# UmbertoDellaMonica/fp-mash

Measured on AMD Instinct MI355X. Metric: bases/s sketched + Mpairs/s dist, k=21 s=1000, 1/2/4/8 MI355X; %HBM roofline, higher is better.
Workload: dtype u64; 1 GPU; n_seqs_per_gpu=10000, seq_len=2000, k=21, s=1000, pairs_per_gpu=100000000, listed_pairs_per_gpu=1000006, full=False

## Files before the change

### fp-mash_amd/csrc/sketch.hip

```cpp
#include "fpm_device.hpp"
#include "fpm_kernels.hpp"
#include "screen_table.hpp"

namespace fpm {

constexpr int kBlock = 256;
constexpr int kSkWpe = 7;
constexpr int kSkWpeThr = 8;
constexpr int kWaves = kBlock / 64;

#ifdef FPM_SKETCH_PHASES
__device__ uint64_t *g_phase;
#define FPM_PHASE_DECL uint64_t ph_[8] = {0, 0, 0, 0, 0, 0, 0, 0}
#define FPM_PHASE(i) do { if (threadIdx.x == 0) ph_[i] = __builtin_amdgcn_s_memtime(); } while (0)
#define FPM_PHASE_FLUSH do { if (threadIdx.x == 0) for (int q_ = 0; q_ < 8; q_++) g_phase[blockIdx.x * 8 + q_] = ph_[q_]; } while (0)
#else
#define FPM_PHASE_DECL do {} while (0)
#define FPM_PHASE(i) do {} while (0)
#define FPM_PHASE_FLUSH do {} while (0)
#endif

__device__ __forceinline__ uint32_t block_exscan(uint32_t v, uint32_t *tmp, uint32_t *total)
{
    const int lane = threadIdx.x & 63, wave = threadIdx.x >> 6;
// ... 9 lines not shown
        uint32_t acc = 0;
        for (int w = 0; w < kWaves; w++) { uint32_t t = tmp[w]; tmp[w] = acc; acc += t; }
        tmp[kWaves] = acc;
    }
    __syncthreads();
    uint32_t ex = tmp[wave] + x - v;
    *total = tmp[kWaves];
    __syncthreads();
    return ex;
}

__device__ __forceinline__ uint32_t lane_prefix(uint64_t m)
{
    return __builtin_amdgcn_mbcnt_hi((uint32_t)(m >> 32), __builtin_amdgcn_mbcnt_lo((uint32_t)m, 0u));
}

template <int P>
__device__ __forceinline__ void write_distinct(const uint64_t *keys, uint32_t nv, uint64_t *row,
                                               uint32_t s, uint32_t *wcnt, uint32_t *total, int tid)
{
    constexpr int E = P / kBlock;
    constexpr int NW = E * kWaves;
    constexpr int PL = (NW + 63) / 64;
    const int lane = tid & 63, wave = tid >> 6;
#pragma unroll
    for (int e = 0; e < E; e++) {
        const uint32_t i = (uint32_t)(e * kBlock + tid);
        const bool f = i < nv && (i == 0 || keys[i] != keys[i - 1]);
        const uint64_t m = __ballot(f);
        if (lane == 0) wcnt[e * kWaves + wave] = (uint32_t)__popcll(m);
    }
    __syncthreads();
    if (tid < 64) {
        uint32_t v[PL], sum = 0;
#pragma unroll
        for (int q = 0; q < PL; q++) {
            const int i = tid * PL + q;
            v[q] = i < NW ? wcnt[i] : 0u;
            sum += v[q];
        }
        uint32_t x = sum;
#pragma unroll
        for (int d = 1; d < 64; d <<= 1) {
            const uint32_t y = __shfl_up(x, d, 64);
            if (lane >= d) x += y;
        }
        uint32_t ex = x - sum;
#pragma unroll
        for (int q = 0; q < PL; q++) {
            const int i = tid * PL + q;
            if (i < NW) wcnt[i] = ex;
            ex += v[q];
        }
        if (tid == 63) wcnt[NW] = x;
    }
    __syncthreads();
    *total = wcnt[NW];
#pragma unroll
    for (int e = 0; e < E; e++) {
        const uint32_t i = (uint32_t)(e * kBlock + tid);
        const uint64_t key = i < nv ? keys[i] : 0ULL;
        const bool f = i < nv && (i == 0 || key != keys[i - 1]);
        const uint64_t m = __ballot(f);
        const uint32_t rank = wcnt[e * kWaves + wave] + lane_prefix(m);
        if (f && rank < s) row[rank] = key;
    }
}

template <int P>
__device__ void bitonic_sort(uint64_t *keys)
{
    const int tid = threadIdx.x;
    for (int ks = 2; ks <= P; ks <<= 1) {
        for (int j = ks >> 1; j > 0; j >>= 1) {
            for (int t = tid; t < P / 2; t += kBlock) {
                int i = ((t & ~(j - 1)) << 1) | (t & (j - 1));
                int l = i + j;
                bool up = (i & ks) == 0;
                uint64_t a = keys[i], b = keys[l];
                if ((a > b) == up) { keys[i] = b; keys[l] = a; }
            }
            __syncthreads();
        }
    }
}

__device__ __forceinline__ uint32_t upper4(uint32_t x)
{
    const uint32_t hi = x & 0x80808080u, lo = x & 0x7f7f7f7fu;
    const uint32_t ge = (lo + 0x1f1f1f1fu) & ~hi;
    const uint32_t le = ~(lo + 0x05050505u) & ~hi;
    const uint32_t m = (ge & le & 0x80808080u) >> 2;
    return x - m;
}

__device__ __forceinline__ uint32_t compl4(uint32_t x)
{
    const uint32_t b1 = (x >> 1) & 0x01010101u;
    return x ^ (b1 * 0x04u + (b1 ^ 0x01010101u) * 0x15u);
}

template <int P>
struct TileImg {
    static constexpr int E = P / kBlock;
    static constexpr int kRcPad = ((E + 15) / 16) * 16;
    static constexpr int kFBytes = ((P + 31 + 15 + 96 + 31) / 32) * 32;
    static constexpr int kRBytes = ((kRcPad + P + 31 + 15 + 96 + 15) / 16) * 16;
    static constexpr int kMaskWords = kFBytes / 32 + 2;
    static constexpr int kBytes = kFBytes + kRBytes + 4 * kMaskWords + 512;
};

template <int P>
__device__ __forceinline__ void tile_stage(const uint8_t *__restrict__ seq, const TileDesc &td,
                                           const SketchKParams &p, uint32_t *img, int tid)
{
    using I = TileImg<P>;
    uint32_t *const fwd_img = img;
    uint32_t *const rc_img = fwd_img + I::kFBytes / 4;
    uint32_t *const badmask = rc_img + I::kRBytes / 4;
    const uint8_t *const alpha = reinterpret_cast<const uint8_t *>(badmask + I::kMaskWords);
    const uint8_t *const compl_tab = alpha + 256;
    const uint32_t n = td.n_bytes;
    const uint32_t a0 = (uint32_t)(td.byte_off & 15);
    const uint8_t *g0 = seq + (td.byte_off - a0);
    const uint32_t nimg = a0 + n;
    const uint32_t rc0 = I::kRcPad + ((16u - (nimg & 15u)) & 15u);
    constexpr int kChunks = I::kFBytes / 16;
    for (int ch = tid; ch < kChunks; ch += kBlock) {
        const uint32_t y0 = (uint32_t)ch * 16;
        uint4 v = make_uint4(0, 0, 0, 0);
        if (y0 < nimg) v = *reinterpret_cast<const uint4 *>(g0 + y0);
        uint32_t w[4] = {v.x, v.y, v.z, v.w};
        uint32_t bad = 0;
#pragma unroll
        for (int q = 0; q < 4; q++) {
            if (!p.preserve_case) w[q] = upper4(w[q]);
#pragma unroll
            for (int b = 0; b < 4; b++) {
                const uint32_t y = y0 + 4 * q + b;
                const bool ok = y >= a0 && y < nimg && alpha[(w[q] >> (8 * b)) & 0xffu];
                bad |= (ok ? 0u : 1u) << (4 * q + b);
            }
        }
        *reinterpret_cast<uint4 *>(&fwd_img[y0 / 4]) = make_uint4(w[0], w[1], w[2], w[3]);
        if (p.canonical && y0 < nimg) {
            const uint32_t zc = rc0 + nimg - 16 - y0;
            uint32_t c[4];
            if (p.compl_acgt) {
#pragma unroll
                for (int q = 0; q < 4; q++) c[q] = compl4(w[q]);
            } else {
#pragma unroll
                for (int q = 0; q < 4; q++) {
                    uint32_t x = 0;
#pragma unroll
                    for (int b = 0; b < 4; b++)
                        x |= (uint32_t)compl_tab[(w[q] >> (8 * b)) & 0xffu] << (8 * b);
                    c[q] = x;
                }
            }
            *reinterpret_cast<uint4 *>(&rc_img[zc / 4]) =
                make_uint4(__builtin_bswap32(c[3]), __builtin_bswap32(c[2]),
                           __builtin_bswap32(c[1]), __builtin_bswap32(c[0]));
        }
        const uint32_t hi = __shfl_down(bad, 1, 64);
        if ((ch & 1) == 0) badmask[ch / 2] = bad | (hi << 16);
    }
    if (tid < 2) badmask[I::kMaskWords - 2 + tid] = 0xffffffffu;
}

template <int P, int K, typename Sink>
__device__ __forceinline__ uint32_t tile_hash(const TileDesc &td, const SketchKParams &p,
                                              const uint32_t *img, int tid, Sink &&sink)
{
    using I = TileImg<P>;
    constexpr int E = I::E;
    const uint32_t *const fwd_img = img;
    const uint32_t *const rc_img = fwd_img + I::kFBytes / 4;
    const uint32_t *const badmask = rc_img + I::kRBytes / 4;
    const uint32_t n = td.n_bytes;
    const uint32_t k = K ? (uint32_t)K : p.k;
    const uint32_t a0 = (uint32_t)(td.byte_off & 15);
    const uint32_t nimg = a0 + n;
    const uint32_t rc0 = I::kRcPad + ((16u - (nimg & 15u)) & 15u);
    const uint32_t nk = n >= k ? n - k + 1 : 0;
    const int nw = (k + 3) >> 2;
    const uint32_t tail_mask = (k & 3) ? ((1u << (8 * (k & 3))) - 1u) : 0xffffffffu;
    const uint32_t kmask = (k == 32) ? 0xffffffffu : ((1u << k) - 1u);
    constexpr int KW = K ? (K + 3) / 4 : 8;
    constexpr int W = (E + 3) / 4 + KW + 1;
    uint32_t vbits = 0;
    uint32_t seed;
    asm volatile("s_mov_b32 %0, %1" : "=s"(seed) : "s"(p.seed));
    const uint32_t i0 = (uint32_t)tid * E;
    if (i0 < nk) {
        const uint32_t yb = a0 + i0;
        uint32_t okbits = 0;
        {
            const uint32_t wq = yb >> 5, sh = yb & 31;
            uint64_t bits = ((uint64_t)badmask[wq] | ((uint64_t)badmask[wq + 1] << 32)) >> sh;
            if (sh) bits |= (uint64_t)badmask[wq + 2] << (64 - sh);
#pragma unroll
            for (int e = 0; e < E; e++) {
                const bool ok = i0 + e < nk && (((uint32_t)(bits >> e) & kmask) == 0);
                okbits |= (ok ? 1u : 0u) << e;
            }
        }
        if (okbits) {
            uint32_t S[W];
            {
                const uint32_t q0 = yb >> 2, sh0 = yb & 3;
                uint32_t D[W + 1];
#pragma unroll
                for (int m = 0; m <= W; m++) D[m] = fwd_img[q0 + m];
#pragma unroll
                for (int m = 0; m < W; m++) S[m] = __builtin_amdgcn_alignbyte(D[m + 1], D[m], sh0);
            }
            uint32_t SR[W];
            if (p.canonical) {
                const uint32_t zb = rc0 + n - i0 - k - (E - 1);
                const uint32_t qr = zb >> 2, shr = zb & 3;
                uint32_t D[W + 1];
#pragma unroll
                for (int m = 0; m <= W; m++) D[m] = rc_img[qr + m];
#pragma unroll
                for (int m = 0; m < W; m++) SR[m] = __builtin_amdgcn_alignbyte(D[m + 1], D[m], shr);
            }
#pragma unroll
            for (int e = 0; e < E; e++) {
                if (!(okbits >> e & 1)) continue;
                uint32_t d[8];
#pragma unroll
                for (int m = 0; m < 8; m++)
                    d[m] = (m < nw) ? __builtin_amdgcn_alignbyte(S[(e >> 2) + m + 1], S[(e >> 2) + m],
                                                                 e & 3)
                                    : 0u;
                d[nw - 1] &= tail_mask;
                if (p.canonical) {
                    const int f = E - 1 - e;
                    uint32_t r[8];
#pragma unroll
                    for (int m = 0; m < 8; m++)
                        r[m] = (m < nw) ? __builtin_amdgcn_alignbyte(SR[(f >> 2) + m + 1],
                                                                     SR[(f >> 2) + m], f & 3)
                                        : 0u;
                    r[nw - 1] &= tail_mask;
                    constexpr int NQ = K ? ((K + 3) / 4 + 1) / 2 : 4;
                    bool gt = false, eq = true;
#pragma unroll
                    for (int q = 0; q < NQ; q++) {
                        const uint64_t fq = ((uint64_t)__builtin_bswap32(d[2 * q]) << 32) |
                                            __builtin_bswap32(d[2 * q + 1]);
                        const uint64_t rq = ((uint64_t)__builtin_bswap32(r[2 * q]) << 32) |
                                            __builtin_bswap32(r[2 * q + 1]);
                        gt = gt || (eq && fq > rq);
                        eq = eq && fq == rq;
                    }
                    const int cmp = gt ? 1 : 0;
                    if (cmp > 0) {
#pragma unroll
                        for (int m = 0; m < 8; m++) d[m] = r[m];
                    }
                }
                uint64_t wd[4];
#pragma unroll
                for (int j = 0; j < 4; j++) wd[j] = (uint64_t)d[2 * j] | ((uint64_t)d[2 * j + 1] << 32);
                const uint64_t h = murmur_h1_le32(wd, (int)k, seed);
                sink(e, p.use64 ? h : (h & 0xffffffffULL));
            }
            vbits = okbits;
        }
    }
    return vbits;
}

constexpr int kSurv = 2;
constexpr int kSurvShared = 512;
static_assert(kBlock * kSurv + kSurvShared == (int)kThrTileKeys, "sketch_plan.cpp sizes thr4 by it");
template <int P, int K, bool THR>
__device__ __forceinline__ void sketch_tile(
    const uint8_t *__restrict__ seq, const TileDesc td, SketchKParams p,
    const uint64_t *__restrict__ thr, uint64_t *__restrict__ out, uint32_t *__restrict__ out_count,
    TileDesc *__restrict__ redo, uint32_t *__restrict__ redo_n)
{
    using I = TileImg<P>;
    constexpr int E = I::E;
    constexpr int PS = THR ? kBlock * kSurv + kSurvShared : P;
    constexpr int ES = PS / kBlock;
    constexpr int KW = THR ? (PS > (I::kBytes + 7) / 8 ? PS : (I::kBytes + 7) / 8) : P;
    __shared__ __attribute__((aligned(16))) uint64_t keys[KW];
    static_assert(I::kBytes <= 8 * KW, "staging fits in keys");
    constexpr int kBins = P >= 4096 ? P / 4 : P / 2;
    static_assert(!THR || kBins <= 2 * (kBlock * kSurv + kSurvShared), "bins fit the slots");
    __shared__ uint64_t surv[THR ? kBlock * kSurv + kSurvShared : 1];
    __shared__ uint32_t s_over, s_shared;
    uint32_t *const img = reinterpret_cast<uint32_t *>(keys);
    uint8_t *const alpha = reinterpret_cast<uint8_t *>(img + (I::kFBytes + I::kRBytes) / 4 +
                                                       I::kMaskWords);
    uint8_t *const compl_tab = alpha + 256;
    __shared__ uint32_t scan_tmp[kWaves + 1];
    __shared__ uint32_t wcnt[ES * kWaves + 1];
    __shared__ uint32_t bins_own[THR ? 1 : kBins];
    uint32_t *const bins = THR ? reinterpret_cast<uint32_t *>(surv) : bins_own;
    __shared__ uint32_t big_bucket, s_cut;

    FPM_PHASE_DECL;
    FPM_PHASE(0);
    const int tid = threadIdx.x;

    alpha[tid] = p.alphabet[tid];
    compl_tab[tid] = p.complement[tid];
    if (THR && tid == 0) { s_over = 0; s_shared = 0; }
    __syncthreads();

    tile_stage<P>(seq, td, p, img, tid);
    __syncthreads();
    FPM_PHASE(1);

    uint64_t kr[ES];
    uint32_t vbits;
    uint64_t hmax = p.use64 ? ~0ULL : 0xffffffffULL;
    if constexpr (THR) {
        hmax = min(hmax, thr[td.thr_slot - 1]);
        uint32_t ns = 0;
        tile_hash<P, K>(td, p, img, tid, [&](int, uint64_t h) {
            if (h <= hmax) {
                if (ns < (uint32_t)kSurv) {
                    surv[tid * kSurv + ns] = h;
                    ns++;
                } else {
                    const uint32_t j = atomicAdd(&s_shared, 1u);
                    if (j < (uint32_t)kSurvShared) surv[kBlock * kSurv + j] = h;
                    else s_over = 1;
                }
            }
        });
        uint32_t total;
        uint32_t at = block_exscan(ns, scan_tmp, &total);
        if (s_over) {
            if (tid == 0) redo[atomicAdd(redo_n, 1u)] = td;
            return;
        }
        for (uint32_t i = 0; i < ns; i++) keys[at + i] = surv[tid * kSurv + i];
        const uint32_t nsh = s_shared;
        for (uint32_t i = tid; i < nsh; i += kBlock) keys[total + i] = surv[kBlock * kSurv + i];
        total += nsh;
        __syncthreads();
        if (total <= 64) {
            if (tid < 64) {
                const uint64_t v = tid < total ? keys[tid] : 0;
                const uint32_t vlo = (uint32_t)v, vhi = (uint32_t)(v >> 32);
                bool first = tid < total;
#pragma unroll 1
                for (uint32_t j = 0; j < total; j++) {
                    const uint64_t y = ((uint64_t)(uint32_t)__builtin_amdgcn_readlane((int)vhi, (int)j) << 32) |
                                       (uint32_t)__builtin_amdgcn_readlane((int)vlo, (int)j);
                    first = first && !(j < tid && y == v);
                }
                const uint64_t fm = __builtin_amdgcn_ballot_w64(first);
                uint32_t rank = 0;
#pragma unroll 1
                for (uint32_t j = 0; j < total; j++) {
                    const uint64_t y = ((uint64_t)(uint32_t)__builtin_amdgcn_readlane((int)vhi, (int)j) << 32) |
                                       (uint32_t)__builtin_amdgcn_readlane((int)vlo, (int)j);
                    rank += ((fm >> j) & 1) && y < v ? 1u : 0u;
                }
                if (first && rank < p.s) out[(uint64_t)td.out_row * p.s + rank] = v;
                if (tid == 0) {
                    const uint32_t nd = (uint32_t)__popcll(fm);
                    out_count[td.out_row] = nd < p.s ? nd : p.s;
                }
            }
            return;
        }
        vbits = 0;
#pragma unroll
        for (int e = 0; e < ES; e++) {
            const uint32_t j = (uint32_t)tid + (uint32_t)e * kBlock;
            kr[e] = ~0ULL;
            if (j < total) { kr[e] = keys[j]; vbits |= 1u << e; }
        }
        __syncthreads();
    } else {
#pragma unroll
    for (int e = 0; e < E; e++) kr[e] = ~0ULL;
    vbits = tile_hash<P, K>(td, p, img, tid, [&](int e, uint64_t h) { kr[e] = h; });

    FPM_PHASE(2);
    if (td.thr_slot) {
        hmax = min(hmax, thr[td.thr_slot - 1]);
#pragma unroll
        for (int e = 0; e < E; e++)
            if (kr[e] > hmax) vbits &= ~(1u << e);
        if (E > 1) {
            uint32_t total;
            uint32_t at = block_exscan((uint32_t)__popc(vbits), scan_tmp, &total);
            if (total <= (uint32_t)(kBlock * (E / 2))) {
#pragma unroll
                for (int e = 0; e < E; e++)
                    if (vbits >> e & 1) keys[at++] = kr[e];
                __syncthreads();
                vbits = 0;
#pragma unroll
                for (int e = 0; e < E; e++) {
                    const uint32_t j = (uint32_t)tid + (uint32_t)e * kBlock;
                    if (j < total) { kr[e] = keys[j]; vbits |= 1u << e; }
                }
                __syncthreads();
            }
        }
    }
    }

    constexpr int NB = P >= 4096 ? P / 4 : P / 2;
    constexpr int LB = __builtin_ctz(NB);
    constexpr uint32_t kMaxBucket = 32;
    const uint32_t hbits = hmax ? 64 - __clzll(hmax) : 1;
    const uint32_t bshift = hbits > (uint32_t)LB ? hbits - LB : 0;
    for (int b = tid; b < NB; b += kBlock) bins[b] = 0;
    if (tid == 0) { big_bucket = 0; s_cut = NB; }
    __syncthreads();
#pragma unroll
    for (int e = 0; e < ES; e++)
        if (vbits >> e & 1) atomicAdd(&bins[(uint32_t)(kr[e] >> bshift)], 1u);
    __syncthreads();
    FPM_PHASE(3);
    constexpr int per = NB >= kBlock ? NB / kBlock : 1;
    uint32_t run = 0, bmax = 0;
#pragma unroll
    for (int u = 0; u < per; u++) {
        const int b = tid * per + u;
        const uint32_t c = b < NB ? bins[b] : 0u;
        run += c;
        bmax = max(bmax, c);
    }
    uint32_t nvalid;
    uint32_t acc = block_exscan(run, scan_tmp, &nvalid);
#pragma unroll
    for (int u = 0; u < per; u++) {
        const int b = tid * per + u;
        if (b < NB) {
            const uint32_t c = bins[b];
            bins[b] = acc;
            if (acc < p.s && acc + c >= p.s) s_cut = (uint32_t)b + 1;
            acc += c;
        }
    }
    if (bmax > kMaxBucket) big_bucket = 1;
    __syncthreads();
    const uint32_t cut = big_bucket ? (uint32_t)NB : s_cut;
    const uint32_t nkept = cut < (uint32_t)NB ? bins[cut] : nvalid;
    FPM_PHASE(4);
    uint32_t lo_b = 0, hi_b = cut, nv = nkept;
    for (int pass = 0; pass < 2; pass++) {
        uint32_t bsh = bshift;
        asm volatile("" : "+v"(bsh));
        uint32_t act = 0;
#pragma unroll
        for (int e = 0; e < ES; e++) {
            const uint32_t bk = (uint32_t)(kr[e] >> bsh);
            act |= ((vbits >> e & 1) && bk >= lo_b && bk < hi_b) ? (1u << e) : 0u;
        }
        uint32_t slot[ES];
#pragma unroll
        for (int e = 0; e < ES; e++)
            if (act >> e & 1) {
                slot[e] = atomicAdd(&bins[(uint32_t)(kr[e] >> bsh)], 1u);
                keys[slot[e]] = kr[e];
            }
        __syncthreads();
        FPM_PHASE(5);
        if (!big_bucket) {
#pragma unroll
            for (int e = 0; e < ES; e++)
                if (act >> e & 1) {
                    const uint32_t b = (uint32_t)(kr[e] >> bsh);
                    const uint32_t s0 = b ? bins[b - 1] : 0u, s1 = bins[b];
                    const uint32_t mb = s1 - s0;
                    uint32_t r = 0;
#pragma unroll
                    for (uint32_t u = 0; u < 8; u++) {
                        const uint32_t t = s0 + u;
                        const uint64_t y = keys[t < (uint32_t)PS ? t : (uint32_t)PS - 1];
                        r += (u < mb) & ((y < kr[e]) | ((y == kr[e]) & (t < slot[e])));
                    }
                    for (uint32_t t = s0 + 8; t < s1; t++) {
                        const uint64_t y = keys[t];
                        r += (y < kr[e]) | ((y == kr[e]) & (t < slot[e]));
                    }
                    slot[e] = s0 + r;
                }
            __syncthreads();
#pragma unroll
            for (int e = 0; e < ES; e++)
                if (act >> e & 1) keys[slot[e]] = kr[e];
            __syncthreads();
        } else {
            for (int i = tid; i < PS; i += kBlock)
                if ((uint32_t)i >= nvalid) keys[i] = ~0ULL;
            __syncthreads();
            bitonic_sort<PS>(keys);
        }
        FPM_PHASE(6);

        uint32_t total;
        write_distinct<PS>(keys, nv, out + (uint64_t)td.out_row * p.s, p.s, wcnt, &total, tid);
        if (total >= p.s || hi_b >= (uint32_t)NB) {
            if (tid == 0) out_count[td.out_row] = total < p.s ? total : p.s;
            break;
        }
        lo_b = hi_b;
        hi_b = NB;
        nv = nvalid;
    }
    FPM_PHASE(7);
    FPM_PHASE_FLUSH;
}

template <int P, int K, bool THR = false>
__global__ __launch_bounds__(kBlock) __attribute__((amdgpu_waves_per_eu(THR ? (K ? kSkWpeThr : 6) : P <= 2048 ? kSkWpe : P == 4096 ? 4 : 1))) void sketch_tiles_kernel(
    const uint8_t *__restrict__ seq, const TileDesc *__restrict__ tiles, SketchKParams p,
    const uint64_t *__restrict__ thr, uint64_t *__restrict__ out, uint32_t *__restrict__ out_count,
    TileDesc *__restrict__ redo, uint32_t *__restrict__ redo_n)
{
    sketch_tile<P, K, THR>(seq, tiles[blockIdx.x], p, thr, out, out_count, redo, redo_n);
}

template <int K>
__global__ __launch_bounds__(kBlock) __attribute__((amdgpu_waves_per_eu(3))) void sketch_redo_kernel(
    const uint8_t *__restrict__ seq, const TileDesc *__restrict__ redo,
    const uint32_t *__restrict__ redo_n, SketchKParams p, const uint64_t *__restrict__ thr,
    uint64_t *__restrict__ out, uint32_t *__restrict__ out_count)
{
    const uint32_t n = *redo_n;
    for (uint32_t t = blockIdx.x; t < n; t += gridDim.x) {
        sketch_tile<4096, K, false>(seq, redo[t], p, thr, out, out_count, nullptr, nullptr);
        __syncthreads();
    }
}

__device__ __forceinline__ uint32_t lower_bound_u64(const uint64_t *v, uint32_t n, uint64_t x)
{
    uint32_t lo = 0, hi = n;
    while (lo < hi) { uint32_t m = (lo + hi) >> 1; if (v[m] < x) lo = m + 1; else hi = m; }
    return lo;
}
__device__ __forceinline__ uint32_t upper_bound_u64(const uint64_t *v, uint32_t n, uint64_t x)
{
    uint32_t lo = 0, hi = n;
    while (lo < hi) { uint32_t m = (lo + hi) >> 1; if (v[m] <= x) lo = m + 1; else hi = m; }
    return lo;
}

__global__ __launch_bounds__(kBlock) void merge_kernel(const MergeDesc *__restrict__ descs, uint32_t s)
{
    __shared__ uint32_t scan_tmp[kWaves + 1];
    const MergeDesc md = descs[blockIdx.x];
    const uint32_t la = *md.alen, lb = md.b ? *md.blen : 0;
    uint32_t dups_total = 0;
    uint32_t carry = 0;
    for (uint32_t c0 = 0; c0 < la; c0 += kBlock) {
        uint32_t i = c0 + threadIdx.x;
        uint64_t a = 0; uint32_t pos = 0; uint32_t dup = 0;
        if (i < la) {
            a = md.a[i];
            pos = lb ? lower_bound_u64(md.b, lb, a) : 0;
            dup = (pos < lb && md.b[pos] == a) ? 1u : 0u;
        }
        uint32_t tot;
        uint32_t ex = block_exscan(dup, scan_tmp, &tot);
        if (i < la) {
            uint32_t f = i + pos - (carry + ex);
            if (f < s) md.c[f] = a;
        }
        carry += tot;
    }
    dups_total = carry;
    carry = 0;
    for (uint32_t c0 = 0; c0 < lb; c0 += kBlock) {
        uint32_t j = c0 + threadIdx.x;
        uint64_t b = 0; uint32_t pos = 0; uint32_t dup = 0;
        if (j < lb) {
            b = md.b[j];
            pos = upper_bound_u64(md.a, la, b);
            dup = (pos > 0 && md.a[pos - 1] == b) ? 1u : 0u;
        }
        uint32_t tot;
        uint32_t ex = block_exscan(dup, scan_tmp, &tot);
        if (j < lb && !dup) {
            uint32_t f = j + pos - (carry + ex);
            if (f < s) md.c[f] = b;
        }
        carry += tot;
    }
    if (threadIdx.x == 0) {
        uint32_t u = la + lb - dups_total;
        *md.clen = u < s ? u : s;
    }
}

template <int P>
static hipError_t launch_p(const uint8_t *d_seq, const TileDesc *d_tiles, uint32_t n_tiles,
                           const SketchKParams &p, const uint64_t *d_thr, uint64_t *d_out,
                           uint32_t *d_count, hipStream_t st)
{
    if (n_tiles == 0) return hipSuccess;
    if (p.k == 21)
        hipLaunchKernelGGL((sketch_tiles_kernel<P, 21>), dim3(n_tiles), dim3(kBlock), 0, st,
                           d_seq, d_tiles, p, d_thr, d_out, d_count, nullptr, nullptr);
    else
        hipLaunchKernelGGL((sketch_tiles_kernel<P, 0>), dim3(n_tiles), dim3(kBlock), 0, st,
                           d_seq, d_tiles, p, d_thr, d_out, d_count, nullptr, nullptr);
    return hipGetLastError();
}

hipError_t launch_sketch_tiles_thr(const uint8_t *d_seq, const TileDesc *d_tiles, uint32_t n_tiles,
                                   const SketchKParams &p, const uint64_t *d_thr, uint64_t *d_out,
                                   uint32_t *d_count, TileDesc *d_redo, uint32_t *d_redo_n,
                                   hipStream_t st)
{
    if (n_tiles == 0) return hipSuccess;
    if (p.k == 21)
        hipLaunchKernelGGL((sketch_tiles_kernel<4096, 21, true>), dim3(n_tiles), dim3(kBlock), 0,
                           st, d_seq, d_tiles, p, d_thr, d_out, d_count, d_redo, d_redo_n);
    else
        hipLaunchKernelGGL((sketch_tiles_kernel<4096, 0, true>), dim3(n_tiles), dim3(kBlock), 0,
                           st, d_seq, d_tiles, p, d_thr, d_out, d_count, d_redo, d_redo_n);
    return hipGetLastError();
}

hipError_t launch_sketch_redo(const uint8_t *d_seq, const TileDesc *d_redo, const uint32_t *d_redo_n,
                              uint32_t max_tiles, const SketchKParams &p, const uint64_t *d_thr,
                              uint64_t *d_out, uint32_t *d_count, hipStream_t st)
{
    if (max_tiles == 0) return hipSuccess;
    const uint32_t grid = std::min<uint32_t>(max_tiles, 1024);
    if (p.k == 21)
        hipLaunchKernelGGL((sketch_redo_kernel<21>), dim3(grid), dim3(kBlock), 0, st, d_seq, d_redo,
                           d_redo_n, p, d_thr, d_out, d_count);
    else
        hipLaunchKernelGGL((sketch_redo_kernel<0>), dim3(grid), dim3(kBlock), 0, st, d_seq, d_redo,
                           d_redo_n, p, d_thr, d_out, d_count);
    return hipGetLastError();
}

hipError_t launch_sketch_tiles(int cls, const uint8_t *d_seq, const TileDesc *d_tiles,
                               uint32_t n_tiles, const SketchKParams &p, const uint64_t *d_thr,
                               uint64_t *d_out, uint32_t *d_count, hipStream_t st)
{
    switch (cls) {
    case 0: return launch_p<256>(d_seq, d_tiles, n_tiles, p, d_thr, d_out, d_count, st);
    case 1: return launch_p<512>(d_seq, d_tiles, n_tiles, p, d_thr, d_out, d_count, st);
    case 2: return launch_p<1024>(d_seq, d_tiles, n_tiles, p, d_thr, d_out, d_count, st);
    case 3: return launch_p<2048>(d_seq, d_tiles, n_tiles, p, d_thr, d_out, d_count, st);
    case 4: return launch_p<4096>(d_seq, d_tiles, n_tiles, p, d_thr, d_out, d_count, st);
    case 5: return launch_p<8192>(d_seq, d_tiles, n_tiles, p, d_thr, d_out, d_count, st);
    default: return hipErrorInvalidValue;
    }
}

__device__ __forceinline__ uint32_t lower_bound_row(const uint64_t *__restrict__ v, uint32_t n,
                                                    uint64_t x)
{
    uint32_t lo = 0;
    while (n) {
        const uint32_t h = n >> 1;
        if (v[lo + h] < x) { lo += h + 1; n -= h + 1; }
        else n = h;
    }
    return lo;
}

template <int P>
__global__ __launch_bounds__(kBlock) void sketch_mult_kernel(
    const uint8_t *__restrict__ seq, const TileDesc *__restrict__ tiles, SketchKParams p,
    const uint64_t *__restrict__ rows, const uint32_t *__restrict__ count, int pass,
    uint32_t *__restrict__ mult, unsigned long long *__restrict__ first,
    const uint64_t *__restrict__ ttop)
{
    using I = TileImg<P>;
    constexpr int E = I::E;
    __shared__ __attribute__((aligned(16))) uint32_t img[I::kBytes / 4];
    uint8_t *const alpha = reinterpret_cast<uint8_t *>(img + (I::kFBytes + I::kRBytes) / 4 +
                                                       I::kMaskWords);
    uint8_t *const compl_tab = alpha + 256;
    const TileDesc td = tiles[blockIdx.x];
    const uint32_t g = td.pad;
    const uint32_t ng = count[g];
    const bool full = ng >= p.s;
    if (ng == 0) return;
    if (pass == 1 && (!full || td.byte_off > ttop[g])) return;
    const int tid = threadIdx.x;
    alpha[tid] = p.alphabet[tid];
    compl_tab[tid] = p.complement[tid];
    __syncthreads();
    tile_stage<P>(seq, td, p, img, tid);
    __syncthreads();
    uint64_t kr[E];
#pragma unroll
    for (int e = 0; e < E; e++) kr[e] = ~0ULL;
    const uint32_t vbits = tile_hash<P, 0>(td, p, img, tid, [&](int e, uint64_t h) { kr[e] = h; });
    const uint64_t *row = rows + (uint64_t)g * p.s;
    const uint64_t hmax = row[ng - 1];
    uint32_t *mrow = mult + (uint64_t)g * p.s;
#pragma unroll
    for (int e = 0; e < E; e++) {
        if (!(vbits >> e & 1) || kr[e] > hmax) continue;
        const uint64_t pos = td.byte_off + (uint64_t)tid * E + e;
        if (pass == 0) {
            const uint32_t i = lower_bound_row(row, ng, kr[e]);
            if (row[i] != kr[e]) continue;
            if (!(full && i == ng - 1)) atomicAdd(&mrow[i], 1u);
            atomicMin(&first[(uint64_t)g * p.s + i], (unsigned long long)pos);
        } else if (kr[e] == hmax && pos <= ttop[g]) {
            atomicAdd(&mrow[ng - 1], 1u);
        }
    }
}

__global__ __launch_bounds__(kBlock) void mult_ttop_kernel(const uint32_t *__restrict__ count,
                                                         uint32_t n_groups, uint32_t s,
                                                         const unsigned long long *__restrict__ first,
                                                         uint64_t *__restrict__ ttop)
{
    __shared__ unsigned long long red[kWaves];
    const uint32_t g = blockIdx.x;
    if (g >= n_groups) return;
    const uint32_t ng = count[g];
    unsigned long long m = 0;
    for (uint32_t i = threadIdx.x; i < ng; i += kBlock) m = max(m, first[(uint64_t)g * s + i]);
    for (int o = 32; o; o >>= 1) m = max(m, __shfl_xor(m, o, 64));
    if ((threadIdx.x & 63) == 0) red[threadIdx.x >> 6] = m;
    __syncthreads();
    if (threadIdx.x == 0) {
        for (int w = 1; w < kWaves; w++) m = max(m, red[w]);
        ttop[g] = m;
    }
}

hipError_t launch_sketch_mult(int cls, int pass, const uint8_t *d_seq, const TileDesc *d_tiles,
                              uint32_t n_tiles, const SketchKParams &p, const uint64_t *d_rows,
                              const uint32_t *d_count, uint32_t *d_mult,
                              unsigned long long *d_first, const uint64_t *d_ttop, hipStream_t st)
{
    if (n_tiles == 0) return hipSuccess;
#define FPM_MULT_CASE(c, P)                                                                    \
    case c:                                                                                    \
        hipLaunchKernelGGL((sketch_mult_kernel<P>), dim3(n_tiles), dim3(kBlock), 0, st, d_seq,  \
                           d_tiles, p, d_rows, d_count, pass, d_mult, d_first, d_ttop);         \
        break;
    switch (cls) {
        FPM_MULT_CASE(0, 256)
        FPM_MULT_CASE(1, 512)
        FPM_MULT_CASE(2, 1024)
        FPM_MULT_CASE(3, 2048)
        FPM_MULT_CASE(4, 4096)
        FPM_MULT_CASE(5, 8192)
    default: return hipErrorInvalidValue;
    }
#undef FPM_MULT_CASE
    return hipGetLastError();
}

hipError_t launch_mult_ttop(const uint32_t *d_count, uint32_t n_groups, uint32_t s,
                            const unsigned long long *d_first, uint64_t *d_ttop, hipStream_t st)
{
    if (n_groups == 0) return hipSuccess;
    hipLaunchKernelGGL(mult_ttop_kernel, dim3(n_groups), dim3(kBlock), 0, st, d_count, n_groups,
                       s, d_first, d_ttop);
    return hipGetLastError();
}

template <int P>
__global__ __launch_bounds__(kBlock) void reads_count_kernel(
    const uint8_t *__restrict__ seq, const TileDesc *__restrict__ tiles, SketchKParams p,
    const uint64_t *__restrict__ rows, const uint32_t *__restrict__ count, uint32_t m,
    uint32_t *__restrict__ wcnt, unsigned long long *__restrict__ slots)
{
    using I = TileImg<P>;
    constexpr int E = I::E;
    __shared__ __attribute__((aligned(16))) uint32_t img[I::kBytes / 4];
    uint8_t *const alpha = reinterpret_cast<uint8_t *>(img + (I::kFBytes + I::kRBytes) / 4 +
                                                       I::kMaskWords);
    uint8_t *const compl_tab = alpha + 256;
    const TileDesc td = tiles[blockIdx.x];
    const uint32_t g = td.pad;
    const uint32_t ng = count[g];
    if (ng == 0) return;
    const int tid = threadIdx.x;
    alpha[tid] = p.alphabet[tid];
    compl_tab[tid] = p.complement[tid];
    __syncthreads();
    tile_stage<P>(seq, td, p, img, tid);
    __syncthreads();
    uint64_t kr[E];
#pragma unroll
    for (int e = 0; e < E; e++) kr[e] = ~0ULL;
    const uint32_t vbits = tile_hash<P, 0>(td, p, img, tid, [&](int e, uint64_t h) { kr[e] = h; });
    const uint64_t *row = rows + (uint64_t)g * p.s;
    const uint64_t hmax = row[ng - 1];
#pragma unroll
    for (int e = 0; e < E; e++) {
        if (!(vbits >> e & 1) || kr[e] > hmax) continue;
        const uint32_t i = lower_bound_row(row, ng, kr[e]);
        if (row[i] != kr[e]) continue;
        const uint64_t at = (uint64_t)g * p.s + i;
        atomicAdd(&wcnt[at], 1u);
        unsigned long long x = td.byte_off + (uint64_t)tid * E + e;
        for (uint32_t j = 0; j < m; j++) {
            const unsigned long long old = atomicMin(&slots[at * m + j], x);
            x = max(old, x);
            if (x == ~0ULL) break;
        }
    }
// ... 683 lines not shown
```

Before: 27.92 billion bases/s.

## Scatter all valid keys once and rank-sort by contiguous prefix slices

Valid k-mer hashes are now scattered into bucket order once, before the pass loop, instead of once per pass filtered by bucket range. The in-bucket rank sort then walks a contiguous index range of the staged keys in strided slices across threads, rather than each thread ranking its own register keys under a per-element activity mask. This aims to balance work across lanes and cut divergent loop iterations, since only the kept prefix (about s entries) needs ranking in the first pass. The kept count is now captured in shared memory during the scan, because the scatter now advances the bin offsets before that count would otherwise be read. The trade-off is an extra shared-memory read of each key during ranking, and scattering keys beyond the cut that a single pass would not need.

```diff
diff --git a/fp-mash_amd/csrc/sketch.hip b/fp-mash_amd/csrc/sketch.hip
--- a/fp-mash_amd/csrc/sketch.hip
+++ b/fp-mash_amd/csrc/sketch.hip
@@ -335,7 +335,7 @@
     __shared__ uint32_t wcnt[ES * kWaves + 1];
     __shared__ uint32_t bins_own[THR ? 1 : kBins];
     uint32_t *const bins = THR ? reinterpret_cast<uint32_t *>(surv) : bins_own;
-    __shared__ uint32_t big_bucket, s_cut;
+    __shared__ uint32_t big_bucket, s_cut, s_nkept;
 
     FPM_PHASE_DECL;
     FPM_PHASE(0);
@@ -475,39 +475,33 @@
         if (b < NB) {
             const uint32_t c = bins[b];
             bins[b] = acc;
-            if (acc < p.s && acc + c >= p.s) s_cut = (uint32_t)b + 1;
+            if (acc < p.s && acc + c >= p.s) { s_cut = (uint32_t)b + 1; s_nkept = acc + c; }
             acc += c;
         }
     }
     if (bmax > kMaxBucket) big_bucket = 1;
     __syncthreads();
     const uint32_t cut = big_bucket ? (uint32_t)NB : s_cut;
-    const uint32_t nkept = cut < (uint32_t)NB ? bins[cut] : nvalid;
+    const uint32_t nkept = cut < (uint32_t)NB ? s_nkept : nvalid;
     FPM_PHASE(4);
-    uint32_t lo_b = 0, hi_b = cut, nv = nkept;
+#pragma unroll
+    for (int e = 0; e < ES; e++)
+        if (vbits >> e & 1) keys[atomicAdd(&bins[(uint32_t)(kr[e] >> bshift)], 1u)] = kr[e];
+    __syncthreads();
+    uint32_t lo_p = 0, hi_p = nkept, hi_b = cut, nv = nkept;
     for (int pass = 0; pass < 2; pass++) {
-        uint32_t bsh = bshift;
-        asm volatile("" : "+v"(bsh));
-        uint32_t act = 0;
-#pragma unroll
-        for (int e = 0; e < ES; e++) {
-            const uint32_t bk = (uint32_t)(kr[e] >> bsh);
-            act |= ((vbits >> e & 1) && bk >= lo_b && bk < hi_b) ? (1u << e) : 0u;
-        }
-        uint32_t slot[ES];
-#pragma unroll
-        for (int e = 0; e < ES; e++)
-            if (act >> e & 1) {
-                slot[e] = atomicAdd(&bins[(uint32_t)(kr[e] >> bsh)], 1u);
-                keys[slot[e]] = kr[e];
-            }
-        __syncthreads();
         FPM_PHASE(5);
         if (!big_bucket) {
-#pragma unroll
-            for (int e = 0; e < ES; e++)
-                if (act >> e & 1) {
-                    const uint32_t b = (uint32_t)(kr[e] >> bsh);
+            const uint32_t span = (uint32_t)__builtin_amdgcn_readfirstlane((int)(hi_p - lo_p));
+            uint64_t x[ES];
+            uint32_t dst[ES];
+#pragma unroll
+            for (int i = 0; i < ES; i++) {
+                if ((uint32_t)i * kBlock >= span) break;
+                const uint32_t j = lo_p + (uint32_t)i * kBlock + (uint32_t)tid;
+                if (j < hi_p) {
+                    x[i] = keys[j];
+                    const uint32_t b = (uint32_t)(x[i] >> bshift);
                     const uint32_t s0 = b ? bins[b - 1] : 0u, s1 = bins[b];
                     const uint32_t mb = s1 - s0;
                     uint32_t r = 0;
@@ -515,18 +509,21 @@
                     for (uint32_t u = 0; u < 8; u++) {
                         const uint32_t t = s0 + u;
                         const uint64_t y = keys[t < (uint32_t)PS ? t : (uint32_t)PS - 1];
-                        r += (u < mb) & ((y < kr[e]) | ((y == kr[e]) & (t < slot[e])));
+                        r += (u < mb) & ((y < x[i]) | ((y == x[i]) & (t < j)));
                     }
                     for (uint32_t t = s0 + 8; t < s1; t++) {
                         const uint64_t y = keys[t];
-                        r += (y < kr[e]) | ((y == kr[e]) & (t < slot[e]));
+                        r += (y < x[i]) | ((y == x[i]) & (t < j));
                     }
-                    slot[e] = s0 + r;
+                    dst[i] = s0 + r;
                 }
+            }
             __syncthreads();
 #pragma unroll
-            for (int e = 0; e < ES; e++)
-                if (act >> e & 1) keys[slot[e]] = kr[e];
+            for (int i = 0; i < ES; i++) {
+                if ((uint32_t)i * kBlock >= span) break;
+                if (lo_p + (uint32_t)i * kBlock + (uint32_t)tid < hi_p) keys[dst[i]] = x[i];
+            }
             __syncthreads();
         } else {
             for (int i = tid; i < PS; i += kBlock)
@@ -542,7 +539,8 @@
             if (tid == 0) out_count[td.out_row] = total < p.s ? total : p.s;
             break;
         }
-        lo_b = hi_b;
+        lo_p = nkept;
+        hi_p = nvalid;
         hi_b = NB;
         nv = nvalid;
     }
```

After: 28.67 billion bases/s, median of 6. +2.7%, better.
